# brentyi/multimodalfilter

Measured on AMD Instinct MI355X. Metric: filter steps/sec (batch x particles), higher is better.
Workload: dtype f32 via f16x3 (operands split into 2 f16 halves exact to 2^-22, 3 f16 MFMA products per product, f32 accumulate)

## Files before the change

multimodalfilter_amd/csrc/particle_net.hip:

```cpp
#include <hip/hip_fp16.h>
#include <stdlib.h>

#include <cmath>
#include <cstdio>
#include <vector>

#include <utility>

#include "mmf_common.h"
#include "mmf_launch.h"
#include "../../include/mmf_detmath.h"
#include "../../include/mmf_philox.h"

#include "particle_net_tiles.h"

namespace {

__global__ void pack_particle_net_kernel(MmfParticleNetDesc d, float* __restrict__ out, int precision) {
  const int total = blob_floats(d.n_res);
  for (int q = blockIdx.x * blockDim.x + threadIdx.x; q < total; q += gridDim.x * blockDim.x) {
    float v = 0.f;
    if (q < off_layers()) {
      const int row = q / kW0Cols, k = q % kW0Cols;
      if (k < d.d_in) v = d.w_in[row * d.d_in + k];
// ... 160 lines not shown
    step(std::integral_constant<int, 2>{}); step(std::integral_constant<int, 3>{});
    if constexpr (l > 0) {
      Act<CT>& prev = out_is_h(l - 1) ? H : X;
      act_tile<CT, 1, act_in>(prev);
      split_tile<CT, 1, signed_in>(prev, SP, neg_one, amax);
    }
    pin_small_region<CT, 4, 6>();
    __builtin_amdgcn_sched_barrier(0);
    step(std::integral_constant<int, 4>{}); step(std::integral_constant<int, 5>{});
    if constexpr (l + 1 < NL) {
      constexpr int m = l + 1;
      Act<CT>& nxt = out_is_h(m) ? H : X;
      if constexpr (m == 2) {
        join_init(nxt);
      } else if constexpr (m == 1 || (m > 3 && (m - 3) % 2 == 1)) {
        add_bias_packed<CT>(lds + off_bias(NRES) + m * kUnits, nxt, h);
      } else {
        add_bias<CT, false>(lds + off_bias(NRES) + m * kUnits, nxt, h, 1.f);
      }
    }
    pin_small_region<CT, 2, 6>();
    __builtin_amdgcn_sched_barrier(0);
    step(std::integral_constant<int, 6>{}); step(std::integral_constant<int, 7>{});
    act_tile<CT, 0, act_next>(out);
    if constexpr (l + 1 < NL) split_tile<CT, 0, signed_next>(out, SP, neg_one, amax);
    pin_small_region<CT, 2, 6>();
    __builtin_amdgcn_sched_barrier(0);
    (void)sizeof(I);
  });
  act_tile<CT, 1, kActReluSat>(H);
}



struct NetArgs {
  const float* packed;
  const float* states_in;
  const float* traj_bias;
  const float* noise;
  const float* scale_tril;
  const float* mod_logw;
  float* states_out;
  float* loglik;
  float* jac;
  int R;
  int M;
  int logw_stride;
  int combine;
  int* range_flag;
  unsigned long long noise_seed;
  unsigned noise_step, noise_traj0;
  int noise_mode;
};

#ifdef MMF_K2_WG_STAMPS
__device__ long long g_k2_stamp[2][512];
__device__ int g_k2_xcc[512];
#define K2_WG_STAMP(which)                                                                          \
  do {                                                                                              \
    if (threadIdx.x == 0 && blockIdx.y == 0 && blockIdx.x < 512) {                                  \
      unsigned x_;                                                                                  \
      asm volatile("s_getreg_b32 %0, hwreg(HW_REG_XCC_ID)" : "=s"(x_));                             \
      g_k2_stamp[which][blockIdx.x] = wall_clock64();                                               \
      g_k2_xcc[blockIdx.x] = x_ & 0xf;                                                              \
    }                                                                                               \
  } while (0)
#else
#define K2_WG_STAMP(which)
#endif

struct NetArgsMulti {
  NetArgs a[MMF_LOOP_MAX_MEAS];
};

struct RunTable {
  const int32_t* rank;
  const int32_t* run_anc;
  const int32_t* run_start;
  const int32_t* n_runs;
};
struct NetArgsRuns {
  NetArgs a[1];
  RunTable rt;
};

template <int D, int NRES, int KIND, int CT, int PREC, int WPS, bool PIPE = false, bool RUNS = false>
__global__ __launch_bounds__(WPS * 256, WPS) void particle_net_kernel(std::conditional_t<RUNS, NetArgsRuns, NetArgsMulti> multi) {
  const NetArgs a = multi.a[blockIdx.y];
  static_assert(!RUNS || KIND == kDynamics, "only the dynamics launch consumes a run table");
  K2_WG_STAMP(0);
  static_assert(!PIPE || (CT == 2 && PREC == MMF_PREC_F16X3 && KIND != kJacobian), "pipelined halves: f16x3, 64-particle tiles");
  constexpr int kThreads = WPS * 256;
  constexpr int kWavesPerBlock = kThreads / MMF_WAVE;
  extern __shared__ __attribute__((aligned(16))) float lds[];
  constexpr bool JAC = KIND == kJacobian;
  constexpr bool F16 = PREC == MMF_PREC_F16X3;
  constexpr int NOUT = (KIND == kMeasure) ? 1 : D + 1;
  constexpr int TILE = 32 * CT;
  static_assert(!JAC || D <= 3, "jacobian groups are 4 columns: primal + up to 3 tangents");

#ifdef MMF_K2_SYNC_STAGING
  constexpr bool ASYNC_STAGE = false;
#else
  constexpr bool ASYNC_STAGE = PIPE && kThreads == 512;
#endif
  constexpr int NLAYERS = 3 + 2 * NRES;
  const int lane = threadIdx.x & 63;
  const int j = lane & 31, h = lane >> 5;
  const int wave_global = blockIdx.x * kWavesPerBlock + (threadIdx.x >> 6);
  const int waves_total = gridDim.x * kWavesPerBlock;
  const int ntiles = (a.R + TILE - 1) / TILE;
  if constexpr (!ASYNC_STAGE) {
    const float4* src = reinterpret_cast<const float4*>(a.packed);
    float4* dst = reinterpret_cast<float4*>(lds);
    mmf::stage_to_lds<blob_floats(NRES) / 4, kThreads>(src, dst, threadIdx.x);
    __syncthreads();
  } else {
    const float4* src = reinterpret_cast<const float4*>(a.packed);
    float4* dst = reinterpret_cast<float4*>(lds);
    static_assert(off_layers() % 256 == 0 && off_bias(NRES) % 4 == 0 && blob_floats(NRES) % 4 == 0, "16-byte sections, 1 KB pieces");
    for (int i = threadIdx.x; i < off_layers() / 4; i += kThreads) dst[i] = src[i];
    for (int i = off_bias(NRES) / 4 + threadIdx.x; i < blob_floats(NRES) / 4; i += kThreads) dst[i] = src[i];
  }

  float neg_one = -1.0f;
  asm volatile("" : "+s"(neg_one));

  constexpr int KS0 = (D + 2) / 2;
  const int n_traj = RUNS ? a.R / a.M : 1;
  auto runs_of = [&](int tile, int& q, int& traj) {
    q = tile / n_traj;
    traj = tile - q * n_traj;
    q = (q + traj) % (a.M / TILE);
    int nr = 0;
    if constexpr (RUNS) nr = multi.rt.n_runs[traj];
    nr = nr < 1 ? 1 : (nr > a.M ? a.M : nr);
    return nr;
  };
  auto first_layer_inputs = [&](int tile, float (&b)[KS0][CT]) {
    const int base = tile * TILE;
    int run_q = 0, run_traj = 0, run_n = 0;
    if constexpr (RUNS) run_n = runs_of(tile, run_q, run_traj);
#pragma unroll
    for (int s = 0; s < KS0; ++s) {
      const int comp = 2 * s + h;
#pragma unroll
      for (int c = 0; c < CT; ++c) {
        int row = base + 32 * c + j;
        row = row < a.R ? row : a.R - 1;
        if constexpr (RUNS) {
          int run = run_q * TILE + 32 * c + j;
          run = run < run_n ? run : run_n - 1;
          int anc = multi.rt.run_anc[static_cast<size_t>(run_traj) * (a.M + 1) + run];
          anc = anc < 0 ? 0 : (anc < a.M ? anc : a.M - 1);
          row = run_traj * a.M + anc;
        }
        float v;
        if (JAC) {
          const int role = row & 3;
          if (role == 0) v = comp < D ? a.states_in[(row >> 2) * D + comp] : (comp == D ? 1.f : 0.f);
          else v = (comp == role - 1) ? 1.f : 0.f;
        } else {
          v = comp < D ? a.states_in[static_cast<size_t>(row) * D + comp] : (comp == D ? 1.f : 0.f);
        }
        b[s][c] = v;
      }
    }
  };
  float bnext[KS0][CT];
  auto tile_real = [&](int tile) {
    int q, traj;
    const int nr = runs_of(tile, q, traj);
    return q * TILE < nr;
  };
  bool first_pending = false;
  if constexpr (RUNS) {
    const int t0 = __builtin_amdgcn_readfirstlane(wave_global);
    if (t0 < ntiles) {
      if (tile_real(t0)) first_layer_inputs(t0, bnext);
      else first_pending = true;
    }
  } else {
    if (wave_global < ntiles) first_layer_inputs(wave_global, bnext);
  }
  bool layers_pending = false;
  __shared__ int s_next_index;
  if constexpr (ASYNC_STAGE) {
    if (threadIdx.x == 0) s_next_index = 2 * kWavesPerBlock;
#pragma unroll
    for (int s = 0; s < KS0; ++s)
#pragma unroll
      for (int c = 0; c < CT; ++c) asm volatile("" : "+v"(bnext[s][c]));
    const unsigned lds_base = static_cast<unsigned>(reinterpret_cast<uintptr_t>(lds)) + off_layers() * 4;
    const unsigned char* gsrc = reinterpret_cast<const unsigned char*>(a.packed + off_layers()) + lane * 16;
    const int wv = threadIdx.x >> 6;
#pragma unroll
    for (int l = 0; l < NLAYERS; ++l)
#pragma unroll
      for (int q = 0; q < 2; ++q) {
        const unsigned piece = static_cast<unsigned>(l * 16 + wv * 2 + q) * 1024u;
        const unsigned dst = __builtin_amdgcn_readfirstlane(lds_base + piece);
        const unsigned char* sp = gsrc + piece;
        unsigned keep;
        asm volatile("s_mov_b32 %0, m0\n\ts_mov_b32 m0, %2\n\ts_nop 0\n\tglobal_load_lds_dwordx4 %1, off\n\ts_mov_b32 m0, %0"
                     : "=&s"(keep) : "v"(sp), "s"(dst) : "memory");
      }
    asm volatile("s_waitcnt vmcnt(%0) lgkmcnt(0)" ::"n"(2 * (NLAYERS - 2)) : "memory");
    __builtin_amdgcn_s_barrier();
    asm volatile("" ::: "memory");
    layers_pending = true;
  }
  auto await_layers = [&]() {
    if (layers_pending) {
      asm volatile("s_waitcnt vmcnt(0)" ::: "memory");
      __builtin_amdgcn_s_barrier();
      asm volatile("" ::: "memory");
      layers_pending = false;
    }
  };

  const bool claims = ntiles > 2 * waves_total;
  if constexpr (!ASYNC_STAGE) {
    if (claims) {
      if (threadIdx.x == 0) s_next_index = 2 * kWavesPerBlock;
      __syncthreads();
    }
  }
  auto tile_of = [&](int i) { return (i / kWavesPerBlock) * waves_total + blockIdx.x * kWavesPerBlock + i % kWavesPerBlock; };
  auto claim = [&](int after) {
    if (!claims) return after + kWavesPerBlock;
    int v = 0;
    if (lane == 0) v = atomicAdd(&s_next_index, 1);
    return __builtin_amdgcn_readfirstlane(v);
  };
  int i_next = (threadIdx.x >> 6) + kWavesPerBlock;
  auto advance = [&]() {
    for (;;) {
      const int t = __builtin_amdgcn_readfirstlane(tile_of(i_next));
      i_next = claim(i_next);
      if (t >= ntiles) return t;
      if (tile_real(t)) {
        first_layer_inputs(t, bnext);
        return t;
      }
    }
  };
  int tile_first = wave_global;
  if constexpr (RUNS) {
    tile_first = __builtin_amdgcn_readfirstlane(tile_first);
    if (first_pending) tile_first = advance();
  }

  for (int tile = tile_first; tile < ntiles;) {
    int tile_next = RUNS ? 0 : tile_of(i_next);
    const int base = tile * TILE;
    int run_q = 0, run_traj = 0, run_n = 0;
    if constexpr (RUNS) run_n = runs_of(tile, run_q, run_traj);
    int col_row[CT], col_traj[CT];
    bool col_primal[CT];
#pragma unroll
    for (int c = 0; c < CT; ++c) {
      int row = base + 32 * c + j;
      row = row < a.R ? row : a.R - 1;
      col_row[c] = row;
      col_traj[c] = RUNS ? run_traj : JAC ? (row >> 2) : (row / a.M);
      col_primal[c] = JAC ? ((row & 3) == 0) : true;
    }
    const bool primal = col_primal[0];

    Act<CT> X, H;
    float bcur[KS0][CT];
#pragma unroll
    for (int s = 0; s < KS0; ++s)
#pragma unroll
      for (int c = 0; c < CT; ++c) bcur[s][c] = bnext[s][c];
    if constexpr (RUNS) {
      tile_next = advance();
    } else {
      if (tile_next < ntiles) first_layer_inputs(tile_next, bnext);
      i_next = claim(i_next);
    }
    first_layer<CT>(lds, bcur, X, lane);
    short2v amax = {0, 0};
    if constexpr (F16) seed_nonfinite<CT>(bcur, amax);
    if constexpr (PIPE) {
      constexpr int NL = 3 + 2 * NRES;
      FragPair frag;
      SplitAct<CT> SP;
      relu<CT, false>(X, true);
      auto vstage = [&](auto half, auto layer) {
        constexpr int C = decltype(half)::value;
        constexpr int l = decltype(layer)::value;
        const float* bl = lds + off_bias(NRES) + l * kUnits;
        if constexpr (l == 0) {
          split_half<C, false>(X, SP, neg_one, amax);
          bias_half<C, false>(bl, H, h);
        } else if constexpr (l == 1) {
          relu_half<C>(H);
          split_half<C, false>(H, SP, neg_one, amax);
          bias_half<C, true>(bl, X, h);
        } else if constexpr (l == 2) {
          relu_half<C>(X);
          split_half<C, false>(X, SP, neg_one, amax);
          join_init<CT>(H, C, load_join_row(a.traj_bias + static_cast<size_t>(col_traj[C]) * kUnits, lane));
        } else if constexpr ((l - 3) % 2 == 0) {
          constexpr bool kSigned = (l == 3 && KIND != kMeasure);
          if constexpr (kSigned) saturate_half<C>(H);
          else relu_half<C, (l != 3)>(H);
          split_half<C, kSigned>(H, SP, neg_one, amax);
          bias_half<C, false>(bl, X, h);
        } else {
          relu_half<C>(X);
          split_half<C, false>(X, SP, neg_one, amax);
          bias_half<C, true>(bl, H, h);
        }
      };
      auto mstage = [&](auto half, auto layer) {
        constexpr int C = decltype(half)::value;
        constexpr int l = decltype(layer)::value;
        constexpr bool to_h = (l == 0 || l == 2 || (l > 2 && (l - 3) % 2 == 1));
        constexpr int ln = (C == 0) ? l : (l + 1 < NL ? l + 1 : l);
        mfma_half<C>(lds + off_layers() + l * kLayerFloats, lds + off_layers() + ln * kLayerFloats, frag, SP,
                     to_h ? H : X, lane);
      };
      using I0 = std::integral_constant<int, 0>;
      using I1 = std::integral_constant<int, 1>;
      asm volatile("" ::: "memory");
      frag = load_frag(lds + off_layers(), lane, 0);
      vstage(I0{}, I0{});
      __builtin_amdgcn_sched_barrier(0);
      static_for<NL>([&](auto layer) {
        constexpr int l = decltype(layer)::value;
        mstage(I0{}, layer);
        vstage(I1{}, layer);
        pin_mfma_valu_interleave<5>();
        __builtin_amdgcn_sched_barrier(0);
        if constexpr (ASYNC_STAGE && l == 1) await_layers();
        mstage(I1{}, layer);
        if constexpr (l + 1 < NL) vstage(I0{}, std::integral_constant<int, l + 1>{});
        else relu_half<0>(H);
        pin_mfma_valu_interleave<5>();
        __builtin_amdgcn_sched_barrier(0);
      });
      relu_half<1>(H);
    } else {
      net_unpipelined<CT, NRES, KIND, PREC>(lds, X, H, [&](Act<CT>& acc) {
#pragma unroll
        for (int c = 0; c < CT; ++c)
          join_init<CT>(acc, c, load_join_row(a.traj_bias + static_cast<size_t>(col_traj[c]) * kUnits, lane), !JAC || primal);
      }, lane, neg_one, amax, primal);
    }
    if constexpr (F16) report_range(a.range_flag, amax);

    float out[NOUT][CT];
    head<NRES>(lds, H, lane, out);

    float mine[NOUT];
#pragma unroll
    for (int o = 0; o < NOUT; ++o) {
      if (CT == 2) {
        float lo_col = out[o][0], hi_col = out[o][CT - 1];
        asm volatile("" : "+v"(lo_col), "+v"(hi_col));
        mine[o] = h ? hi_col : lo_col;
      } else {
        mine[o] = out[o][0];
      }
    }
    const int my_row = base + (CT == 2 ? lane : j);
    const bool active = my_row < a.R && (CT == 2 || h == 0);
    const float* bh = lds + off_bhead(NRES);

    if constexpr (KIND == kMeasure) {
      if (active) {
        const int traj = my_row / a.M;
        float ll = mine[0] + bh[0];
        if (a.mod_logw) ll += a.mod_logw[static_cast<size_t>(traj) * a.logw_stride];
        if (a.combine) {
          const float prev = a.loglik[my_row];
          if constexpr (PREC == MMF_PREC_F32) {
            ll = mmf_det_logaddexp(prev, ll);
          } else {
            const float m = fmaxf(prev, ll);
            ll = (m == -INFINITY) ? m : m + logf(expf(prev - m) + expf(ll - m));
          }
        }
        a.loglik[my_row] = ll;
      }
    } else if constexpr (KIND == kDynamics && RUNS) {
      const size_t tab = static_cast<size_t>(run_traj) * (a.M + 1);
      const int r0 = run_q * TILE;
      const int r1 = r0 + TILE < run_n ? r0 + TILE : run_n;
      int my_run = r0 + (CT == 2 ? lane : j);
      my_run = my_run < run_n ? my_run : run_n - 1;
      int anc = multi.rt.run_anc[tab + my_run];
      anc = anc < 0 ? 0 : (anc < a.M ? anc : a.M - 1);
      float xo[D], v0[D];
#pragma unroll
      for (int i = 0; i < D; ++i) xo[i] = a.states_in[(static_cast<size_t>(run_traj) * a.M + anc) * D + i];
      dynamics_drift<D, PREC>(mine, bh, xo, v0);
      int s0 = multi.rt.run_start[tab + r0], s1 = multi.rt.run_start[tab + r1];
      s0 = s0 < 0 ? 0 : s0;
      s1 = s1 > a.M ? a.M : s1;
      const bool noisy = a.noise != nullptr || a.noise_mode == 2;
      for (int kb = s0; kb < s1; kb += MMF_WAVE) {
        const int k = kb + lane;
        const bool live = k < s1;
        const int kk = live ? k : s1 - 1;
        const size_t slot = static_cast<size_t>(run_traj) * a.M + kk;
        const int src = multi.rt.rank[slot] - r0;
        float v[D], eps[D], xn[D];
#pragma unroll
        for (int i = 0; i < D; ++i) {
          v[i] = __shfl(v0[i], src);
          eps[i] = (a.noise_mode != 2 && a.noise) ? a.noise[slot * D + i] : 0.f;
        }
        dynamics_diffuse<D>(v, eps, a.scale_tril, noisy, a.noise_mode == 2, a.noise_seed, a.noise_step,
                            a.noise_traj0 + static_cast<unsigned>(run_traj), static_cast<unsigned>(kk), xn);
        if (live) {
#pragma unroll
          for (int i = 0; i < D; ++i) a.states_out[slot * D + i] = xn[i];
        }
      }
    } else if constexpr (KIND == kDynamics) {
      if (active) {
        float xo[D], eps[D], xn[D];
#pragma unroll
        for (int i = 0; i < D; ++i) {
          xo[i] = a.states_in[static_cast<size_t>(my_row) * D + i];
          eps[i] = (a.noise_mode != 2 && a.noise) ? a.noise[static_cast<size_t>(my_row) * D + i] : 0.f;
        }
        const unsigned traj = static_cast<unsigned>(my_row / a.M);
        dynamics_update<D, PREC>(mine, bh, xo, eps, a.scale_tril, a.noise != nullptr || a.noise_mode == 2, a.noise_mode == 2,
                                 a.noise_seed, a.noise_step, a.noise_traj0 + traj, static_cast<unsigned>(my_row) - traj * a.M, xn);
#pragma unroll
        for (int i = 0; i < D; ++i) a.states_out[static_cast<size_t>(my_row) * D + i] = xn[i];
      }
    } else {
      if constexpr (CT == 1 || F16) {
        const int role = my_row & 3;
        const int traj = my_row >> 2;
        float dirp[D], gatep;
#pragma unroll
        for (int i = 0; i < D; ++i) dirp[i] = quad_first(mine[i] + bh[i]);
        gatep = quad_first(mine[D] + bh[D]);
        const float sg = 1.0f / (1.0f + expf(-gatep));
        if (active) {
          if (role == 0) {
#pragma unroll
            for (int i = 0; i < D; ++i)
              a.states_out[traj * D + i] = jac_primal(a.states_in[traj * D + i], dirp[i], sg);
          } else if (role <= D) {
            const float dgate = mine[D];
#pragma unroll
            for (int i = 0; i < D; ++i) {
              const float dv = jac_tangent(mine[i], sg, dirp[i], dgate, (i == role - 1) ? 1.f : 0.f);
              a.jac[(static_cast<size_t>(traj) * D + i) * D + (role - 1)] = dv;
            }
          }
        }
      } else {
        const int my_col = my_row < a.R ? my_row : a.R - 1;
        const int role = my_col & 3;
        const int traj = my_col >> 2;
        float x[D], own[D];
#pragma unroll
        for (int i = 0; i < D; ++i) x[i] = role == 0 ? a.states_in[traj * D + i] : 0.f;
        jacobian_outputs<D>(mine, bh, x, role, own);
        float* dst = role == 0 ? a.states_out + traj * D : a.jac + static_cast<size_t>(traj) * D * D + (role - 1);
        const int stride = role == 0 ? 1 : D;
        if (active && role <= D) {
#pragma unroll
          for (int i = 0; i < D; ++i) dst[i * stride] = own[i];
        }
      }
    }
    tile = tile_next;
  }
  if constexpr (ASYNC_STAGE) await_layers();
  K2_WG_STAMP(1);
}

template <int D, int NRES, int KIND, int PREC, int CT, int WPS, bool PIPE = false>
int launch_variant(const NetArgsMulti& m, int count, hipStream_t s) {
  const NetArgs& a = m.a[0];
  const size_t lds = static_cast<size_t>(blob_floats(NRES)) * sizeof(float);
  constexpr int waves = WPS * 4, tile = 32 * CT;
  const int ntiles = (a.R + tile - 1) / tile;
  int grid = (ntiles + waves - 1) / waves;
  if (grid > 256) grid = 256;
  if (grid < 1) grid = 1;
  auto k = particle_net_kernel<D, NRES, KIND, CT, PREC, WPS, PIPE>;
  return mmf::launch(k, dim3(grid, count), WPS * 256, lds, s, m);
}

template <int D, int NRES, int KIND, int PREC>
int launch_ct(const NetArgsMulti& m, int count, hipStream_t s) {
  const NetArgs& a = m.a[0];
  const bool big = a.R >= 256 * 8 * 64;
  if constexpr (PREC == MMF_PREC_F16X3 && KIND != kJacobian) {
    if (big) return launch_variant<D, NRES, KIND, PREC, 2, 2, true>(m, count, s);
  }
  if (big) return launch_variant<D, NRES, KIND, PREC, 2, 2>(m, count, s);
  return launch_variant<D, NRES, KIND, PREC, 1, 2>(m, count, s);
}

template <int D, int PREC, int CT, bool PIPE>
int launch_runs_variant(const NetArgsRuns& m, hipStream_t s) {
  constexpr int NRES = 3, WPS = 2;
  const size_t lds = static_cast<size_t>(blob_floats(NRES)) * sizeof(float);
  constexpr int waves = WPS * 4, tile = 32 * CT;
  const int ntiles = m.a[0].R / tile;
  int grid = (ntiles + waves - 1) / waves;
  if (grid > 256) grid = 256;
  if (grid < 1) grid = 1;
  auto k = particle_net_kernel<D, NRES, kDynamics, CT, PREC, WPS, PIPE, true>;
  return mmf::launch(k, dim3(grid, 1), WPS * 256, lds, s, m);
}

template <int D>
int launch_runs(const NetArgsRuns& m, int precision, hipStream_t s) {
  const bool big = m.a[0].R >= 256 * 8 * 64;
  if (precision == MMF_PREC_F16X3) {
    if (big) return launch_runs_variant<D, MMF_PREC_F16X3, 2, true>(m, s);
    return launch_runs_variant<D, MMF_PREC_F16X3, 1, false>(m, s);
  }
  if (precision == MMF_PREC_F32) {
    if (big) return launch_runs_variant<D, MMF_PREC_F32, 2, false>(m, s);
    return launch_runs_variant<D, MMF_PREC_F32, 1, false>(m, s);
  }
  return MMF_EINVAL;
}

int dynamics_runs(const float* packed, int n_res, int precision, const float* states_prev, const float* traj_bias,
                  const float* noise, const float* scale_tril, const int32_t* rank, const int32_t* run_anc,
                  const int32_t* run_start, const int32_t* n_runs, float* states_out, int* range_flag, int N, int M, int d,
                  unsigned long long seed, unsigned step, unsigned traj0, int noise_mode, void* stream) {
  if (!packed || !states_prev || !traj_bias || !states_out || !rank || !run_anc || !run_start || !n_runs) return MMF_EINVAL;
  if (states_out == states_prev || ((noise || noise_mode == 2) && !scale_tril)) return MMF_EINVAL;
  if (N < 0 || M < 1 || M % 64 != 0 || n_res != 3) return MMF_EINVAL;
  if (static_cast<long long>(N) * M > 0x7fffffffLL / 8) return MMF_ETOOLARGE;
  if (N == 0) return 0;
  NetArgsRuns m{};
  NetArgs& a = m.a[0];
  a.packed = packed; a.states_in = states_prev; a.traj_bias = traj_bias; a.noise = noise;
  a.scale_tril = scale_tril; a.states_out = states_out; a.R = N * M; a.M = M;
  a.range_flag = range_flag;
  a.noise_seed = seed; a.noise_step = step; a.noise_traj0 = traj0; a.noise_mode = noise_mode;
  m.rt = RunTable{rank, run_anc, run_start, n_runs};
  if (d == 2) return launch_runs<2>(m, precision, static_cast<hipStream_t>(stream));
  if (d == 3) return launch_runs<3>(m, precision, static_cast<hipStream_t>(stream));
  return MMF_EINVAL;
}

template <int KIND>
int launch_multi(const NetArgsMulti& m, int count, int d, int n_res, int precision, hipStream_t s);

template <int KIND>
int launch(const NetArgs& a, int d, int n_res, int precision, hipStream_t s) {
  NetArgsMulti m{};
  m.a[0] = a;
  return launch_multi<KIND>(m, 1, d, n_res, precision, s);
}

template <int KIND>
int launch_multi(const NetArgsMulti& m, int count, int d, int n_res, int precision, hipStream_t s) {
#define MMF_CASE(D, NR)                                                              \
  if (d == D && n_res == NR) {                                                       \
    if (precision == MMF_PREC_F32) return launch_ct<D, NR, KIND, MMF_PREC_F32>(m, count, s); \
    if (precision == MMF_PREC_F16X3) return launch_ct<D, NR, KIND, MMF_PREC_F16X3>(m, count, s); \
    return MMF_EINVAL;                                                               \
  }
  if constexpr (KIND == kJacobian || KIND == kDynamics) {
    MMF_CASE(2, 3) MMF_CASE(3, 3)
  } else {
    MMF_CASE(2, 2) MMF_CASE(3, 2)
  }
#undef MMF_CASE
  return MMF_EINVAL;
}

}

#ifdef MMF_K2_WG_STAMPS
extern "C" int mmf_debug_k2_stamps(long long* stamps , int* xcc ) {
  if (hipDeviceSynchronize() != hipSuccess) return MMF_EINVAL;
  if (hipMemcpyFromSymbol(stamps, HIP_SYMBOL(g_k2_stamp), sizeof(long long) * 1024) != hipSuccess) return MMF_EINVAL;
  return hipMemcpyFromSymbol(xcc, HIP_SYMBOL(g_k2_xcc), sizeof(int) * 512) == hipSuccess ? 0 : MMF_EINVAL;
}
#endif

extern "C" size_t mmf_particle_net_floats(int n_res) {
  if (n_res < 0 || n_res > MMF_MAX_RES) return 0;
  return static_cast<size_t>(blob_floats(n_res));
}

extern "C" int mmf_pack_particle_net(const MmfParticleNetDesc* d, float* packed, int precision,
                                     void* stream) {
  if (!d || !packed) return MMF_EINVAL;
  if (precision != MMF_PREC_F32 && precision != MMF_PREC_F16X3 && precision != MMF_PREC_F16X3_DUAL) return MMF_EINVAL;
  if (d->d_in < 1 || d->d_in > MMF_MAX_STATE_DIM || d->n_res < 0 || d->n_res > MMF_MAX_RES) return MMF_EINVAL;
  if (d->n_out < 1 || d->n_out > kHeadRows) return MMF_EINVAL;
  if (d->join_state_off < 0 || d->join_state_off + kUnits > d->join_in) return MMF_EINVAL;
  if (!d->w_in || !d->b_in || !d->w_join || !d->w_head || !d->b_head) return MMF_EINVAL;
  for (int i = 0; i < 2; ++i)
    if (!d->w_enc[i] || !d->b_enc[i]) return MMF_EINVAL;
  for (int i = 0; i < 2 * d->n_res; ++i)
    if (!d->w_res[i] || !d->b_res[i]) return MMF_EINVAL;
  const int total = blob_floats(d->n_res);
  pack_particle_net_kernel<<<(total + 255) / 256, 256, 0, static_cast<hipStream_t>(stream)>>>(*d, packed, precision);
  MMF_CHECK_LAUNCH();
  return 0;
}

extern "C" int mmf_pf_dynamics(const float* packed, int n_res, int precision, const float* states_in,
                               const float* traj_bias, const float* noise, const float* scale_tril,
                               float* states_out, int* range_flag, int N, int M, int d, void* stream) {
  if (!packed || !states_in || !traj_bias || !states_out || (noise && !scale_tril)) return MMF_EINVAL;
  if (N < 0 || M < 1) return MMF_EINVAL;
  if (static_cast<long long>(N) * M > 0x7fffffffLL / 8) return MMF_ETOOLARGE;
  if (N == 0) return 0;
  NetArgs a{};
  a.packed = packed; a.states_in = states_in; a.traj_bias = traj_bias; a.noise = noise;
  a.scale_tril = scale_tril; a.states_out = states_out; a.R = N * M; a.M = M;
  a.range_flag = range_flag;
  return launch<kDynamics>(a, d, n_res, precision, static_cast<hipStream_t>(stream));
}

extern "C" int mmf_pf_dynamics_philox(const float* packed, int n_res, int precision, const float* states_in,
                                      const float* traj_bias, unsigned long long seed, unsigned step, unsigned traj0,
                                      const float* scale_tril, float* states_out, int* range_flag, int N, int M, int d,
                                      void* stream) {
// ... 141 lines not shown
```

multimodalfilter_amd/_abi.py:

```python
import ctypes
import os
from ctypes import POINTER, Structure, c_float, c_int, c_int32, c_size_t, c_uint64, c_void_p

import torch

_HERE = os.path.dirname(os.path.abspath(__file__))
LIB_PATH = os.environ.get("MMF_LIB_PATH") or os.path.join(_HERE, "libmmf_hip.so")

MMF_UNITS = 64
MMF_MAX_RES = 3
MMF_MAX_STATE_DIM = 4
ABI_VERSION = 42
KIND_DYNAMICS, KIND_MEASURE, KIND_JACOBIAN = 0, 1, 2
PREC_F32, PREC_F16X3, PREC_BF16, PREC_F16X3_DUAL = 0, 1, 2, 3
PRECISIONS = {"f32": PREC_F32, "f16x3": PREC_F16X3}
IMAGE_PRECISIONS = {"f32": PREC_F32, "f16x3": PREC_F16X3, "bf16": PREC_BF16}
FLAG_RANGE, FLAG_GAVE_UP, FLAG_NOT_PD = 1, 4, 16

_FP = c_void_p


class MmfParticleNetDesc(Structure):
    _fields_ = [
        ("d_in", c_int32), ("n_res", c_int32), ("relu_after_join", c_int32), ("n_out", c_int32),
# ... 632 lines not shown
def traj_program(prog: torch.Tensor, n_instr: int, weights: torch.Tensor, io_tensors, R: int,
                 n_slots: int = TRAJ_SLOTS, vec_width: int = 128):
    arr = (c_void_p * TRAJ_MAX_IO)(*[ptr(t) for t in io_tensors] + [None] * (TRAJ_MAX_IO - len(io_tensors)))
    with _on(weights):
        _check(load().mmf_traj_program(ptr(prog, dtype=torch.uint8), n_instr, ptr(weights), arr, R,
                                       n_slots, vec_width, stream_of(weights)), "mmf_traj_program")


def pf_train_finalize(args: MmfPfTrainFinalizeArgs, like: torch.Tensor):
    with _on(like):
        _check(load().mmf_pf_train_finalize(ctypes.byref(args), stream_of(like)), "mmf_pf_train_finalize")


def traj_pack(desc: torch.Tensor, n_desc: int, blob: torch.Tensor):
    with _on(blob):
        _check(load().mmf_traj_pack(ptr(desc, dtype=torch.uint8), n_desc, ptr(blob), stream_of(blob)), "mmf_traj_pack")


def traj_weight_grads(desc: torch.Tensor, n_desc: int, stash: torch.Tensor, dz: torch.Tensor, grads: torch.Tensor,
                      partials, n_slices: int, R: int):
    with _on(grads):
        _check(load().mmf_traj_weight_grads(ptr(desc, dtype=torch.uint8), n_desc, ptr(stash), stash.shape[1], ptr(dz),
                                            dz.shape[1], ptr(grads), grads.numel(), ptr(partials), n_slices, R,
                                            stream_of(grads)), "mmf_traj_weight_grads")


def fc64_train_forward(x, w, b, y):
    R, K = x.shape
    partial = torch.empty((max(1, K // 512), R, 64), dtype=torch.float32, device=x.device)
    with _on(x):
        _check(load().mmf_fc64_train_forward(ptr(x), ptr(w), ptr(b), ptr(y), ptr(partial), R, K, stream_of(x)),
               "mmf_fc64_train_forward")


def fc64_train_backward(g, x, w, dx, dw, db):
    R, K = x.shape
    with _on(x):
        _check(load().mmf_fc64_train_backward(ptr(g), ptr(x), ptr(w), ptr(dx), ptr(dw), ptr(db), R, K, stream_of(x)),
               "mmf_fc64_train_backward")


def pf_reweight_backward(logw_out, states, g_estimate, g_logw_out, d_a, d_states):
    N, M, d = states.shape
    with _on(states):
        _check(load().mmf_pf_reweight_backward(ptr(logw_out), ptr(states), ptr(g_estimate), ptr(g_logw_out), ptr(d_a),
                                               ptr(d_states), N, M, d, stream_of(states)), "mmf_pf_reweight_backward")


def pf_init_particles(mean, covariance, eps, states, logw, not_pd):
    N, M, d = eps.shape
    with _on(eps):
        _check(load().mmf_pf_init_particles(ptr(mean), ptr(covariance), ptr(eps), ptr(states), ptr(logw),
                                            ptr(not_pd, dtype=torch.int32), N, M, d, stream_of(eps)),
               "mmf_pf_init_particles")


def pf_dedup_plan(M: int, d: int, resample_mode: int, soft_alpha: float = 0.0, recording: bool = False) -> bool:
    return load().mmf_pf_dedup_plan(int(M), int(d), int(resample_mode), float(soft_alpha), int(bool(recording))) == 1


def pf_dedup_workspace_words(N: int, M: int) -> int:
    return int(load().mmf_pf_dedup_workspace_words(int(N), int(M)))


def pf_dedup_workspace(words: torch.Tensor, N: int, M: int):
    assert words.dtype == torch.int32 and words.is_contiguous() and words.numel() >= N * M + 2 * N * (M + 1) + N
    ws = MmfPfDedupWorkspace()
    base, o1, o2, o3 = words.data_ptr(), N * M, N * M + N * (M + 1), N * M + 2 * N * (M + 1)
    ws.rank, ws.run_anc, ws.run_start, ws.n_runs = base, base + 4 * o1, base + 4 * o2, base + 4 * o3
    return ws


def pf_resample_runs(loglik, logw_in, states, u, estimate, indices_out, rank, run_anc, run_start, n_runs, *,
                     logw_out=None, cov=None, ess=None, log_evidence=None):
    N, M, d = states.shape
    i32 = torch.int32
    with _on(states):
        _check(load().mmf_pf_resample_runs(ptr(loglik), ptr(logw_in), ptr(states), ptr(u), ptr(estimate), ptr(logw_out),
                                           ptr(indices_out, dtype=i32), ptr(rank, dtype=i32), ptr(run_anc, dtype=i32),
                                           ptr(run_start, dtype=i32), ptr(n_runs, dtype=i32), N, M, d, ptr(cov), ptr(ess),
                                           ptr(log_evidence), stream_of(states)), "mmf_pf_resample_runs")


def pf_forward_loop(args: MmfPfLoopArgs, like: torch.Tensor, events=None, event_stride: int = 1, *,
                    ess_threshold: float = None, resampled_steps=None, dedup: MmfPfDedupWorkspace = None,
                    history: MmfPfHistory = None) -> int:
    loc = c_int32(0)
    args.final_location = ctypes.pointer(loc)
    if events is not None:
        arr = (c_void_p * len(events))(*[e.cuda_event for e in events])
        args.events = arr
        args.event_stride = event_stride
    with _on(like):
        if history is not None:
            _check(load().mmf_pf_forward_loop_history(
                ctypes.byref(args), ctypes.byref(history), 0.0 if ess_threshold is None else float(ess_threshold),
                ptr(resampled_steps, dtype=torch.int32), None if dedup is None else ctypes.byref(dedup), stream_of(like)),
                "mmf_pf_forward_loop_history")
        elif ess_threshold is not None:
            _check(load().mmf_pf_forward_loop_adaptive(ctypes.byref(args), float(ess_threshold),
                                                       ptr(resampled_steps, dtype=torch.int32), stream_of(like)),
                   "mmf_pf_forward_loop_adaptive")
        elif dedup is not None:
            _check(load().mmf_pf_forward_loop_dedup(ctypes.byref(args), ctypes.byref(dedup), stream_of(like)),
                   "mmf_pf_forward_loop_dedup")
        else:
            _check(load().mmf_pf_forward_loop(ctypes.byref(args), stream_of(like)), "mmf_pf_forward_loop")
    return int(loc.value)


def pf_smooth_lds_bytes(M: int) -> int:
    return int(load().mmf_pf_smooth_lds_bytes(int(M)))


def pf_smooth(states_steps, loglik_steps, logw_in_steps, logw_in0, indices_steps, lag: int, mean, cov=None, unique=None):
    T, N, M, d = states_steps.shape
    assert loglik_steps.shape == (T, N, M) and mean.shape == (T, N, d)
    assert logw_in_steps is None or logw_in_steps.shape == (T, N, M)
    assert logw_in0 is None or logw_in0.shape == (N, M)
    assert indices_steps is None or indices_steps.shape == (T, N, M)
    assert cov is None or cov.shape == (T, N, d, d)
    assert unique is None or unique.shape == (T, N)
    a = MmfPfSmoothArgs()
    a.T, a.N, a.M, a.d, a.lag = T, N, M, d, int(lag)
    a.states_steps, a.loglik_steps, a.logw_in_steps, a.logw_in0 = vp(states_steps), vp(loglik_steps), vp(logw_in_steps), vp(logw_in0)
    a.indices_steps, a.mean, a.cov, a.unique = vp(indices_steps, torch.int32), vp(mean), vp(cov), vp(unique, torch.int32)
    with _on(states_steps):
        _check(load().mmf_pf_smooth(ctypes.byref(a), stream_of(states_steps)), "mmf_pf_smooth")
```

Baseline: 2.273 billion.

## Schedule dedup dynamics tiles densely via per-trajectory prefix sum of run counts

Measured after the change: 2.295 billion (median of 6 runs). No clear change (+1.0%).

```diff
diff --git a/multimodalfilter_amd/csrc/particle_net.hip b/multimodalfilter_amd/csrc/particle_net.hip
--- a/multimodalfilter_amd/csrc/particle_net.hip
+++ b/multimodalfilter_amd/csrc/particle_net.hip
@@ -266,6 +266,15 @@
 struct NetArgsRuns {
   NetArgs a[1];
   RunTable rt;
+  int dense;
+};
+
+constexpr size_t kDensePrefixBytes = 10u << 10;
+static_assert(static_cast<size_t>(blob_floats(3)) * sizeof(float) + kDensePrefixBytes + 256 <= mmf::kLdsPerCu, "P behind the dynamics blob");
+constexpr bool dense_schedule_fits(int n_traj) { return (static_cast<size_t>(n_traj) + 1) * sizeof(int32_t) <= kDensePrefixBytes; }
+
+struct RunTile {
+  int q, traj, n;
 };
 
 template <int D, int NRES, int KIND, int CT, int PREC, int WPS, bool PIPE = false, bool RUNS = false>
@@ -293,7 +302,45 @@
   const int j = lane & 31, h = lane >> 5;
   const int wave_global = blockIdx.x * kWavesPerBlock + (threadIdx.x >> 6);
   const int waves_total = gridDim.x * kWavesPerBlock;
-  const int ntiles = (a.R + TILE - 1) / TILE;
+  int ntiles = (a.R + TILE - 1) / TILE;
+  [[maybe_unused]] int* const s_prefix = reinterpret_cast<int*>(lds + blob_floats(NRES));
+  [[maybe_unused]] bool dense = false;
+  [[maybe_unused]] RunTile dense_first{0, 0, 1};
+  if constexpr (RUNS) {
+    dense = multi.dense != 0;
+    if (dense) {
+      const int n_traj = a.R / a.M;
+      const int t0 = __builtin_amdgcn_readfirstlane(wave_global);
+      const bool writer = threadIdx.x < MMF_WAVE;
+      int sum = 0, traj0 = 0, p0 = 0, n0 = 1;
+      for (int base = 0; base < n_traj; base += 4 * MMF_WAVE) {
+        int nr[4];
+#pragma unroll
+        for (int u = 0; u < 4; ++u) {
+          const int i = base + u * MMF_WAVE + lane;
+          nr[u] = i < n_traj ? multi.rt.n_runs[i] : 1;
+        }
+#pragma unroll
+        for (int u = 0; u < 4; ++u) {
+          const int i = base + u * MMF_WAVE + lane;
+          const int n = nr[u] < 1 ? 1 : (nr[u] > a.M ? a.M : nr[u]);
+          const unsigned nt = i < n_traj ? static_cast<unsigned>((n + TILE - 1) / TILE) : 0u;
+          const int incl = sum + static_cast<int>(mmf::wave_inclusive_scan_u32(nt));
+          if (writer && i < n_traj) s_prefix[i + 1] = incl;
+          const int before = __builtin_popcountll(__builtin_amdgcn_ballot_w64(i < n_traj && incl <= t0));
+          const int in_chunk = n_traj - (base + u * MMF_WAVE);
+          if (before > 0) p0 = __builtin_amdgcn_readlane(incl, before - 1);
+          if (in_chunk > 0 && before < MMF_WAVE && before < in_chunk && traj0 == base + u * MMF_WAVE)
+            n0 = __builtin_amdgcn_readlane(n, before);
+          traj0 += before;
+          sum = __builtin_amdgcn_readlane(incl, MMF_WAVE - 1);
+        }
+      }
+      if (threadIdx.x == 0) s_prefix[0] = 0;
+      ntiles = sum;
+      dense_first = RunTile{t0 - p0, traj0, n0};
+    }
+  }
   if constexpr (!ASYNC_STAGE) {
     const float4* src = reinterpret_cast<const float4*>(a.packed);
     float4* dst = reinterpret_cast<float4*>(lds);
@@ -312,19 +359,31 @@
 
   constexpr int KS0 = (D + 2) / 2;
   const int n_traj = RUNS ? a.R / a.M : 1;
-  auto runs_of = [&](int tile, int& q, int& traj) {
-    q = tile / n_traj;
-    traj = tile - q * n_traj;
-    q = (q + traj) % (a.M / TILE);
+  auto locate = [&](int tile) {
+    RunTile r{0, 0, 0};
+    if (dense) {
+      const int i1 = lane * MMF_WAVE;
+      const int p1 = s_prefix[i1 <= n_traj ? i1 : n_traj];
+      const int c = __builtin_popcountll(__builtin_amdgcn_ballot_w64(i1 <= n_traj && p1 <= tile)) - 1;
+      const int i2 = c * MMF_WAVE + lane;
+      const int p2 = s_prefix[i2 <= n_traj ? i2 : n_traj];
+      const int k = __builtin_popcountll(__builtin_amdgcn_ballot_w64(i2 <= n_traj && p2 <= tile)) - 1;
+      r.traj = c * MMF_WAVE + k;
+      r.traj = r.traj < n_traj ? r.traj : n_traj - 1;
+      r.q = tile - __builtin_amdgcn_readlane(p2, k);
+    } else {
+      r.q = tile / n_traj;
+      r.traj = tile - r.q * n_traj;
+      r.q = (r.q + r.traj) % (a.M / TILE);
+    }
     int nr = 0;
-    if constexpr (RUNS) nr = multi.rt.n_runs[traj];
-    nr = nr < 1 ? 1 : (nr > a.M ? a.M : nr);
-    return nr;
+    if constexpr (RUNS) nr = multi.rt.n_runs[r.traj];
+    r.n = nr < 1 ? 1 : (nr > a.M ? a.M : nr);
+    return r;
   };
-  auto first_layer_inputs = [&](int tile, float (&b)[KS0][CT]) {
+  auto first_layer_inputs = [&](int tile, float (&b)[KS0][CT], const RunTile rt = RunTile{0, 0, 0}) {
     const int base = tile * TILE;
-    int run_q = 0, run_traj = 0, run_n = 0;
-    if constexpr (RUNS) run_n = runs_of(tile, run_q, run_traj);
+    const int run_q = rt.q, run_traj = rt.traj, run_n = rt.n;
 #pragma unroll
     for (int s = 0; s < KS0; ++s) {
       const int comp = 2 * s + h;
@@ -352,16 +411,14 @@
     }
   };
   float bnext[KS0][CT];
-  auto tile_real = [&](int tile) {
-    int q, traj;
-    const int nr = runs_of(tile, q, traj);
-    return q * TILE < nr;
-  };
+  [[maybe_unused]] RunTile rt_next{0, 0, 0};
+  auto tile_real = [&](const RunTile& r) { return r.q * TILE < r.n; };
   bool first_pending = false;
   if constexpr (RUNS) {
     const int t0 = __builtin_amdgcn_readfirstlane(wave_global);
     if (t0 < ntiles) {
-      if (tile_real(t0)) first_layer_inputs(t0, bnext);
+      rt_next = dense ? dense_first : locate(t0);
+      if (tile_real(rt_next)) first_layer_inputs(t0, bnext, rt_next);
       else first_pending = true;
     }
   } else {
@@ -423,8 +480,10 @@
       const int t = __builtin_amdgcn_readfirstlane(tile_of(i_next));
       i_next = claim(i_next);
       if (t >= ntiles) return t;
-      if (tile_real(t)) {
-        first_layer_inputs(t, bnext);
+      const RunTile r = locate(t);
+      if (tile_real(r)) {
+        rt_next = r;
+        first_layer_inputs(t, bnext, r);
         return t;
       }
     }
@@ -438,8 +497,7 @@
   for (int tile = tile_first; tile < ntiles;) {
     int tile_next = RUNS ? 0 : tile_of(i_next);
     const int base = tile * TILE;
-    int run_q = 0, run_traj = 0, run_n = 0;
-    if constexpr (RUNS) run_n = runs_of(tile, run_q, run_traj);
+    const int run_q = rt_next.q, run_traj = rt_next.traj, run_n = rt_next.n;
     int col_row[CT], col_traj[CT];
     bool col_primal[CT];
 #pragma unroll
@@ -691,7 +749,8 @@
 template <int D, int PREC, int CT, bool PIPE>
 int launch_runs_variant(const NetArgsRuns& m, hipStream_t s) {
   constexpr int NRES = 3, WPS = 2;
-  const size_t lds = static_cast<size_t>(blob_floats(NRES)) * sizeof(float);
+  size_t lds = static_cast<size_t>(blob_floats(NRES)) * sizeof(float);
+  if (m.dense) lds += (static_cast<size_t>(m.a[0].R / m.a[0].M) + 1) * sizeof(int32_t);
   constexpr int waves = WPS * 4, tile = 32 * CT;
   const int ntiles = m.a[0].R / tile;
   int grid = (ntiles + waves - 1) / waves;
@@ -731,6 +790,8 @@
   a.range_flag = range_flag;
   a.noise_seed = seed; a.noise_step = step; a.noise_traj0 = traj0; a.noise_mode = noise_mode;
   m.rt = RunTable{rank, run_anc, run_start, n_runs};
+  static const bool dense_enabled = !(getenv("MMF_PF_DEDUP_DENSE") && getenv("MMF_PF_DEDUP_DENSE")[0] == '0');
+  m.dense = dense_enabled && dense_schedule_fits(N);
   if (d == 2) return launch_runs<2>(m, precision, static_cast<hipStream_t>(stream));
   if (d == 3) return launch_runs<3>(m, precision, static_cast<hipStream_t>(stream));
   return MMF_EINVAL;
```

## Prefetch run metadata and per-tile n_runs probe into LDS for dedup dynamics

Applied to the files above, without the earlier changes.

Result: faster. 2.251 billion before, 2.276 billion after, median of 6 (+1.1%).

```diff
diff --git a/multimodalfilter_amd/_abi.py b/multimodalfilter_amd/_abi.py
--- a/multimodalfilter_amd/_abi.py
+++ b/multimodalfilter_amd/_abi.py
@@ -738,6 +738,28 @@
                                            ptr(log_evidence), stream_of(states)), "mmf_pf_resample_runs")
 
 
+def pf_dynamics_runs(packed, n_res, precision, states_prev, traj_bias, noise, scale_tril, rank, run_anc, run_start, n_runs,
+                     states_out, range_flag, N, M, d):
+    i32 = torch.int32
+    with _on(states_prev):
+        _check(load().mmf_pf_dynamics_runs(ptr(packed), n_res, precision, ptr(states_prev), ptr(traj_bias), ptr(noise),
+                                           ptr(scale_tril), ptr(rank, dtype=i32), ptr(run_anc, dtype=i32),
+                                           ptr(run_start, dtype=i32), ptr(n_runs, dtype=i32), ptr(states_out),
+                                           ptr(range_flag, dtype=i32), N, M, d, stream_of(states_prev)),
+               "mmf_pf_dynamics_runs")
+
+
+def pf_dynamics_runs_philox(packed, n_res, precision, states_prev, traj_bias, seed, step, traj0, scale_tril, rank, run_anc,
+                            run_start, n_runs, states_out, range_flag, N, M, d):
+    i32 = torch.int32
+    with _on(states_prev):
+        _check(load().mmf_pf_dynamics_runs_philox(ptr(packed), n_res, precision, ptr(states_prev), ptr(traj_bias), seed, step,
+                                                  traj0, ptr(scale_tril), ptr(rank, dtype=i32), ptr(run_anc, dtype=i32),
+                                                  ptr(run_start, dtype=i32), ptr(n_runs, dtype=i32), ptr(states_out),
+                                                  ptr(range_flag, dtype=i32), N, M, d, stream_of(states_prev)),
+               "mmf_pf_dynamics_runs_philox")
+
+
 def pf_forward_loop(args: MmfPfLoopArgs, like: torch.Tensor, events=None, event_stride: int = 1, *,
                     ess_threshold: float = None, resampled_steps=None, dedup: MmfPfDedupWorkspace = None,
                     history: MmfPfHistory = None) -> int:
diff --git a/multimodalfilter_amd/csrc/particle_net.hip b/multimodalfilter_amd/csrc/particle_net.hip
--- a/multimodalfilter_amd/csrc/particle_net.hip
+++ b/multimodalfilter_amd/csrc/particle_net.hip
@@ -294,10 +294,45 @@
   const int wave_global = blockIdx.x * kWavesPerBlock + (threadIdx.x >> 6);
   const int waves_total = gridDim.x * kWavesPerBlock;
   const int ntiles = (a.R + TILE - 1) / TILE;
+  auto tile_of = [&](int i) { return (i / kWavesPerBlock) * waves_total + blockIdx.x * kWavesPerBlock + i % kWavesPerBlock; };
+  constexpr int kProbeRegs = 4;
+  constexpr int kProbeCap = kProbeRegs * kThreads;
+  static_assert(!RUNS || (blob_floats(NRES) + kProbeCap + 4) * sizeof(float) <= mmf::kLdsPerCu, "the probe list shares a CU's LDS with the blob");
+  const int n_traj = RUNS ? a.R / a.M : 1;
+  auto clamp_runs = [&](int nr) { return nr < 1 ? 1 : (nr > a.M ? a.M : nr); };
+  const int probe_len = RUNS ? (ntiles + waves_total - 1) / waves_total * kWavesPerBlock : 0;
+  const bool probe_lds = RUNS && probe_len <= kProbeCap;
+  int* probe = nullptr;
+  int probe_val[kProbeRegs];
+  if constexpr (RUNS) {
+    __shared__ int s_probe[kProbeCap];
+    probe = s_probe;
+    if (probe_lds) {
+#pragma unroll
+      for (int r = 0; r < kProbeRegs; ++r) {
+        probe_val[r] = 0;
+        if (r * kThreads < probe_len) {
+          const int i = r * kThreads + static_cast<int>(threadIdx.x);
+          const int t = tile_of(i);
+          if (i < probe_len && t < ntiles) probe_val[r] = multi.rt.n_runs[t % n_traj];
+        }
+      }
+    }
+  }
+  auto publish_probe = [&]() {
+    if (probe_lds) {
+#pragma unroll
+      for (int r = 0; r < kProbeRegs; ++r) {
+        const int i = r * kThreads + static_cast<int>(threadIdx.x);
+        if (i < probe_len) probe[i] = clamp_runs(probe_val[r]);
+      }
+    }
+  };
   if constexpr (!ASYNC_STAGE) {
     const float4* src = reinterpret_cast<const float4*>(a.packed);
     float4* dst = reinterpret_cast<float4*>(lds);
     mmf::stage_to_lds<blob_floats(NRES) / 4, kThreads>(src, dst, threadIdx.x);
+    if constexpr (RUNS) publish_probe();
     __syncthreads();
   } else {
     const float4* src = reinterpret_cast<const float4*>(a.packed);
@@ -305,26 +340,49 @@
     static_assert(off_layers() % 256 == 0 && off_bias(NRES) % 4 == 0 && blob_floats(NRES) % 4 == 0, "16-byte sections, 1 KB pieces");
     for (int i = threadIdx.x; i < off_layers() / 4; i += kThreads) dst[i] = src[i];
     for (int i = off_bias(NRES) / 4 + threadIdx.x; i < blob_floats(NRES) / 4; i += kThreads) dst[i] = src[i];
+    if constexpr (RUNS) publish_probe();
   }
 
   float neg_one = -1.0f;
   asm volatile("" : "+s"(neg_one));
 
   constexpr int KS0 = (D + 2) / 2;
-  const int n_traj = RUNS ? a.R / a.M : 1;
-  auto runs_of = [&](int tile, int& q, int& traj) {
+  auto run_tile = [&](int tile, int& q, int& traj) {
     q = tile / n_traj;
     traj = tile - q * n_traj;
     q = (q + traj) % (a.M / TILE);
+  };
+  auto runs_of = [&](int tile, int& q, int& traj) {
+    run_tile(tile, q, traj);
     int nr = 0;
     if constexpr (RUNS) nr = multi.rt.n_runs[traj];
-    nr = nr < 1 ? 1 : (nr > a.M ? a.M : nr);
-    return nr;
+    return clamp_runs(nr);
   };
-  auto first_layer_inputs = [&](int tile, float (&b)[KS0][CT]) {
+  int anc_next = 0, slots_next = 0;
+  auto first_layer_inputs = [&](int tile, float (&b)[KS0][CT], int run_n = 0) {
     const int base = tile * TILE;
-    int run_q = 0, run_traj = 0, run_n = 0;
-    if constexpr (RUNS) run_n = runs_of(tile, run_q, run_traj);
+    int run_q = 0, run_traj = 0;
+    int run_row[CT];
+    if constexpr (RUNS) {
+      run_tile(tile, run_q, run_traj);
+      const size_t tab = static_cast<size_t>(run_traj) * (a.M + 1);
+#pragma unroll
+      for (int c = 0; c < CT; ++c) {
+        int run = run_q * TILE + 32 * c + j;
+        run = run < run_n ? run : run_n - 1;
+        int anc = multi.rt.run_anc[tab + run];
+        anc = anc < 0 ? 0 : (anc < a.M ? anc : a.M - 1);
+        run_row[c] = anc;
+      }
+      int lo_col = run_row[0], hi_col = run_row[CT - 1];
+      asm volatile("" : "+v"(lo_col), "+v"(hi_col));
+      anc_next = h ? hi_col : lo_col;
+      const int r0 = run_q * TILE;
+      const int r1 = r0 + TILE < run_n ? r0 + TILE : run_n;
+      slots_next = multi.rt.run_start[tab + ((lane & 1) ? r1 : r0)];
+#pragma unroll
+      for (int c = 0; c < CT; ++c) run_row[c] += run_traj * a.M;
+    }
 #pragma unroll
     for (int s = 0; s < KS0; ++s) {
       const int comp = 2 * s + h;
@@ -332,13 +390,7 @@
       for (int c = 0; c < CT; ++c) {
         int row = base + 32 * c + j;
         row = row < a.R ? row : a.R - 1;
-        if constexpr (RUNS) {
-          int run = run_q * TILE + 32 * c + j;
-          run = run < run_n ? run : run_n - 1;
-          int anc = multi.rt.run_anc[static_cast<size_t>(run_traj) * (a.M + 1) + run];
-          anc = anc < 0 ? 0 : (anc < a.M ? anc : a.M - 1);
-          row = run_traj * a.M + anc;
-        }
+        if constexpr (RUNS) row = run_row[c];
         float v;
         if (JAC) {
           const int role = row & 3;
@@ -352,16 +404,14 @@
     }
   };
   float bnext[KS0][CT];
-  auto tile_real = [&](int tile) {
-    int q, traj;
-    const int nr = runs_of(tile, q, traj);
-    return q * TILE < nr;
-  };
+  auto tile_real = [&](int q, int nr) { return q * TILE < nr; };
   bool first_pending = false;
   if constexpr (RUNS) {
     const int t0 = __builtin_amdgcn_readfirstlane(wave_global);
     if (t0 < ntiles) {
-      if (tile_real(t0)) first_layer_inputs(t0, bnext);
+      int q, traj;
+      const int nr = runs_of(t0, q, traj);
+      if (tile_real(q, nr)) first_layer_inputs(t0, bnext, nr);
       else first_pending = true;
     }
   } else {
@@ -375,6 +425,7 @@
     for (int s = 0; s < KS0; ++s)
 #pragma unroll
       for (int c = 0; c < CT; ++c) asm volatile("" : "+v"(bnext[s][c]));
+    if constexpr (RUNS) asm volatile("" : "+v"(anc_next), "+v"(slots_next));
     const unsigned lds_base = static_cast<unsigned>(reinterpret_cast<uintptr_t>(lds)) + off_layers() * 4;
     const unsigned char* gsrc = reinterpret_cast<const unsigned char*>(a.packed + off_layers()) + lane * 16;
     const int wv = threadIdx.x >> 6;
@@ -410,7 +461,6 @@
       __syncthreads();
     }
   }
-  auto tile_of = [&](int i) { return (i / kWavesPerBlock) * waves_total + blockIdx.x * kWavesPerBlock + i % kWavesPerBlock; };
   auto claim = [&](int after) {
     if (!claims) return after + kWavesPerBlock;
     int v = 0;
@@ -420,11 +470,16 @@
   int i_next = (threadIdx.x >> 6) + kWavesPerBlock;
   auto advance = [&]() {
     for (;;) {
-      const int t = __builtin_amdgcn_readfirstlane(tile_of(i_next));
+      const int i = i_next;
+      const int t = __builtin_amdgcn_readfirstlane(tile_of(i));
       i_next = claim(i_next);
       if (t >= ntiles) return t;
-      if (tile_real(t)) {
-        first_layer_inputs(t, bnext);
+      int q, traj;
+      run_tile(t, q, traj);
+      int nr = 0;
+      if constexpr (RUNS) nr = probe_lds ? __builtin_amdgcn_readfirstlane(probe[i]) : clamp_runs(multi.rt.n_runs[traj]);
+      if (tile_real(q, nr)) {
+        first_layer_inputs(t, bnext, nr);
         return t;
       }
     }
@@ -438,8 +493,8 @@
   for (int tile = tile_first; tile < ntiles;) {
     int tile_next = RUNS ? 0 : tile_of(i_next);
     const int base = tile * TILE;
-    int run_q = 0, run_traj = 0, run_n = 0;
-    if constexpr (RUNS) run_n = runs_of(tile, run_q, run_traj);
+    int run_q = 0, run_traj = 0;
+    if constexpr (RUNS) run_tile(tile, run_q, run_traj);
     int col_row[CT], col_traj[CT];
     bool col_primal[CT];
 #pragma unroll
@@ -458,8 +513,27 @@
     for (int s = 0; s < KS0; ++s)
 #pragma unroll
       for (int c = 0; c < CT; ++c) bcur[s][c] = bnext[s][c];
+    int slot_lo = 0, slot_hi = 0, rank_first = 0;
+    float xo_mine[D], eps_first[D];
     if constexpr (RUNS) {
+      const int anc_mine = anc_next, slots = slots_next;
       tile_next = advance();
+      slot_lo = __builtin_amdgcn_readlane(slots, 0);
+      slot_hi = __builtin_amdgcn_readlane(slots, 1);
+      slot_lo = slot_lo < 0 ? 0 : slot_lo;
+      slot_hi = slot_hi > a.M ? a.M : slot_hi;
+#pragma unroll
+      for (int i = 0; i < D; ++i) {
+        xo_mine[i] = a.states_in[(static_cast<size_t>(run_traj) * a.M + anc_mine) * D + i];
+        eps_first[i] = 0.f;
+      }
+      if (slot_lo < slot_hi) {
+        const int k = slot_lo + lane;
+        const size_t slot = static_cast<size_t>(run_traj) * a.M + (k < slot_hi ? k : slot_hi - 1);
+        rank_first = multi.rt.rank[slot];
+#pragma unroll
+        for (int i = 0; i < D; ++i) eps_first[i] = (a.noise_mode != 2 && a.noise) ? a.noise[slot * D + i] : 0.f;
+      }
     } else {
       if (tile_next < ntiles) first_layer_inputs(tile_next, bnext);
       i_next = claim(i_next);
@@ -571,33 +645,29 @@
         a.loglik[my_row] = ll;
       }
     } else if constexpr (KIND == kDynamics && RUNS) {
-      const size_t tab = static_cast<size_t>(run_traj) * (a.M + 1);
       const int r0 = run_q * TILE;
-      const int r1 = r0 + TILE < run_n ? r0 + TILE : run_n;
-      int my_run = r0 + (CT == 2 ? lane : j);
-      my_run = my_run < run_n ? my_run : run_n - 1;
-      int anc = multi.rt.run_anc[tab + my_run];
-      anc = anc < 0 ? 0 : (anc < a.M ? anc : a.M - 1);
-      float xo[D], v0[D];
-#pragma unroll
-      for (int i = 0; i < D; ++i) xo[i] = a.states_in[(static_cast<size_t>(run_traj) * a.M + anc) * D + i];
-      dynamics_drift<D, PREC>(mine, bh, xo, v0);
-      int s0 = multi.rt.run_start[tab + r0], s1 = multi.rt.run_start[tab + r1];
-      s0 = s0 < 0 ? 0 : s0;
-      s1 = s1 > a.M ? a.M : s1;
+      float v0[D];
+      dynamics_drift<D, PREC>(mine, bh, xo_mine, v0);
+      const int s0 = slot_lo, s1 = slot_hi;
       const bool noisy = a.noise != nullptr || a.noise_mode == 2;
+      int slot_rank = rank_first;
+      float eps[D];
+#pragma unroll
+      for (int i = 0; i < D; ++i) eps[i] = eps_first[i];
       for (int kb = s0; kb < s1; kb += MMF_WAVE) {
         const int k = kb + lane;
         const bool live = k < s1;
         const int kk = live ? k : s1 - 1;
         const size_t slot = static_cast<size_t>(run_traj) * a.M + kk;
-        const int src = multi.rt.rank[slot] - r0;
-        float v[D], eps[D], xn[D];
-#pragma unroll
-        for (int i = 0; i < D; ++i) {
-          v[i] = __shfl(v0[i], src);
-          eps[i] = (a.noise_mode != 2 && a.noise) ? a.noise[slot * D + i] : 0.f;
+        if (kb != s0) {
+          slot_rank = multi.rt.rank[slot];
+#pragma unroll
+          for (int i = 0; i < D; ++i) eps[i] = (a.noise_mode != 2 && a.noise) ? a.noise[slot * D + i] : 0.f;
         }
+        const int src = slot_rank - r0;
+        float v[D], xn[D];
+#pragma unroll
+        for (int i = 0; i < D; ++i) v[i] = __shfl(v0[i], src);
         dynamics_diffuse<D>(v, eps, a.scale_tril, noisy, a.noise_mode == 2, a.noise_seed, a.noise_step,
                             a.noise_traj0 + static_cast<unsigned>(run_traj), static_cast<unsigned>(kk), xn);
         if (live) {
```
